# luliic2/rttnw

Measured on NVIDIA B200. Metric: path samples/sec, higher is better.
Workload: dtype f64

## Files before the change

rttnw_b200/csrc/api.cu:

```cuda
#include <cuda_runtime.h>
#include <dlfcn.h>

#include <cmath>
#include <cstdio>
#include <cstdlib>
#include <cstring>
#include <mutex>
#include <algorithm>
#include <chrono>
#include <condition_variable>
#include <deque>
#include <functional>
#include <thread>
#include <new>
#include <string>
#include <vector>

#include "../../include/rttnw_b200.h"
#include "flatten.hpp"
#include "adaptive.cuh"
#include "kernels.cuh"
#include "lbvh.cuh"
#include "sah_build.cuh"
#include "shade2.cuh"
#include "trace2.cuh"
#include "trace3.cuh"
#include "scene_api.hpp"

namespace {

thread_local std::string g_err = "";

int fail(int code, const std::string& msg) {
    g_err = msg;
    return code;
// ... 10 lines not shown

struct ArenaSlot {
    void* p;
    size_t bytes;
};
struct ArraySlot {
    cudaArray_t arr;
    cudaTextureObject_t tex;
    int w, h;
};
struct DeviceCache {
    std::mutex m;
    std::vector<ArenaSlot> arenas;
    std::vector<ArraySlot> arrays;
};
constexpr int kMaxDevices = 64;
constexpr size_t kCacheKeep = 4;
DeviceCache g_cache[kMaxDevices];

}

struct rtx_ctx {
    int device = 0;
    cudaStream_t stream = nullptr;
    bool own_stream = false;
    int sm_count = 0;
    unsigned int* d_work_counter = nullptr;
    rtx::Counters* d_counters = nullptr;
    int node_burst = 4;
    int mode = 1;
    void* d_pool = nullptr;
    int pool_slots = 0, pool_slots_wanted = 1 << 19;
    unsigned long long* d_next_item = nullptr;
    unsigned int* d_active = nullptr;
    unsigned long long* h_status = nullptr;
    cudaEvent_t batch_done[8] = {nullptr, nullptr, nullptr, nullptr, nullptr, nullptr, nullptr, nullptr};
    int wf_batch = 8;
    int wf_wide = 0;
    int wf_streams = 2;
    int trace_form = 1;
    int trace_threads = 896;
    int t_leaf = 8, t_refill = 16, t_burst = 8;
    int order_form = 0;
    int order_groups = 512;
    void* d_order = nullptr;
    size_t order_bytes = 0;
    int smem_optin = 0;
    int prof_stride = 8;
    bool perlin_smem = true;
    bool debug_batches = false;
    int shade_form = 2;
    std::vector<cudaStream_t> aux_streams;
    std::vector<cudaEvent_t> join_events;
    cudaEvent_t fork_event = nullptr;
    unsigned long long wf_iterations = 0;
    unsigned long long launches = 0;
    int bvh_builder = 0;
    int ploc_radius = 16;
    int last_build_passes = 0;
    uint8_t* h_stage = nullptr;
    size_t stage_bytes = 0;
    bool profiling = false;
    std::vector<cudaEvent_t> prof_events;
    double prof_shade_ms = 0, prof_trace_ms = 0;
    unsigned long long prof_iterations = 0;
    int w_node = 1, w_leaf = 1, w_shade = 1;
// ... 116 lines not shown
    c->shade_form = env_int("RTX_SHADE", c->shade_form);
    c->debug_batches = env_int("RTX_DEBUG_BATCHES", 0) != 0;
    if (const char* v = std::getenv("RTX_PERLIN_SMEM")) c->perlin_smem = std::atoi(v) != 0;
    c->prof_stride = env_int("RTX_PROF_STRIDE", c->prof_stride);
    if (const char* v = std::getenv("RTX_ORDER")) c->order_form = std::atoi(v);
    c->order_groups = env_int("RTX_ORDER_GROUPS", c->order_groups);
    { int g = 8; while (g * 2 <= c->order_groups && g < (1 << 15)) g *= 2; c->order_groups = g; }
    cudaDeviceGetAttribute(&c->smem_optin, cudaDevAttrMaxSharedMemoryPerBlockOptin, device);
    if (const char* m = std::getenv("RTX_MODE")) c->mode = std::strcmp(m, "mega") == 0 ? 0 : 1;
    if (const char* m = std::getenv("RTX_BVH"))
        c->bvh_builder = std::strcmp(m, "lbvh") == 0 ? 1 : (std::strcmp(m, "ploc") == 0 ? 2 : (std::strcmp(m, "sah_device") == 0 ? 3 : 0));
    c->ploc_radius = env_int("RTX_PLOC_RADIUS", c->ploc_radius);
    cudaFuncSetCacheConfig(rtx::render_kernel<false>, cudaFuncCachePreferL1);
    cudaFuncSetCacheConfig(rtx::trace_rays_kernel<false>, cudaFuncCachePreferL1);
    *out = c;
    return RTX_OK;
}

int rtx_ctx_destroy(rtx_ctx* c) {
    if (!c) return RTX_OK;
    if (c->worker.joinable()) {
        join_async(c);
        { std::lock_guard<std::mutex> lock(c->mu); c->stop = true; }
        c->cv.notify_all();
        c->worker.join();
    }
    cudaSetDevice(c->device);
    if (c->stream || !c->own_stream) cudaStreamSynchronize(c->stream);
    cudaFree(c->d_work_counter);
    cudaFree(c->d_counters);
    cudaFree(c->d_pool);
    cudaFree(c->d_order);
    cudaFree(c->d_next_item);
    cudaFree(c->d_active);
    if (c->h_status) cudaFreeHost(c->h_status);
    if (c->h_stage) cudaFreeHost(c->h_stage);
    for (auto& e : c->batch_done)
        if (e) cudaEventDestroy(e);
    for (auto e : c->prof_events) cudaEventDestroy(e);
    for (auto e : c->join_events) cudaEventDestroy(e);
    for (auto st : c->aux_streams) cudaStreamDestroy(st);
    if (c->fork_event) cudaEventDestroy(c->fork_event);
    if (c->own_stream) cudaStreamDestroy(c->stream);
    delete c;
    return RTX_OK;
}

int rtx_ctx_set_async(rtx_ctx* c, int on) {
    if (!c) return fail(RTX_ERR_INVALID, "ctx is NULL");
    JOIN(c);
    c->async = on != 0;
    if (c->async && !c->worker.joinable()) c->worker = std::thread(worker_main, c);
    return RTX_OK;
}

int rtx_ctx_sync(rtx_ctx* c) {
    if (!c) return fail(RTX_ERR_INVALID, "ctx is NULL");
    JOIN(c);
    CU(cudaSetDevice(c->device));
    CU(cudaStreamSynchronize(c->stream));
    return RTX_OK;
}
void* rtx_ctx_stream(rtx_ctx* c) { return c ? (void*)c->stream : nullptr; }
int rtx_ctx_set_profiling(rtx_ctx* c, int on) {
    if (!c) return fail(RTX_ERR_INVALID, "ctx is NULL");
    c->profiling = on != 0;
// ... 350 lines not shown

int rtx_trace_rays_stats(rtx_ctx* c, const rtx_scene* s, int64_t n, const rtx_ray* d_rays, rtx_trace_stats* out) {
    if (!c || !s || n <= 0 || !d_rays || !out) return fail(RTX_ERR_INVALID, "bad argument");
    JOIN(c);
    CU(cudaSetDevice(c->device));
    CU(cudaMemsetAsync(c->d_counters, 0, sizeof(rtx::Counters), c->stream));
    const int block = 128;
    int64_t grid = (n + block - 1) / block;
    if (grid > 0x7fffffff) return fail(RTX_ERR_INVALID, "too many rays for one launch");
    rtx::trace_rays_kernel<true><<<(unsigned)grid, block, 0, c->stream>>>(s->view, n, d_rays, nullptr, c->d_counters);
    c->launches += 1;
    CU(cudaGetLastError());
    rtx::Counters h;
    CU(cudaMemcpyAsync(&h, c->d_counters, sizeof(h), cudaMemcpyDeviceToHost, c->stream));
    CU(cudaStreamSynchronize(c->stream));
    double dn = (double)n;
    out->rays = dn;
    out->box_tests = (double)h.box_tests / dn;
    out->node_visits = (double)h.node_visits / dn;
    out->sphere_tests = (double)h.sphere_tests / dn;
    out->rect_tests = (double)h.rect_tests / dn;
    out->instance_enters = (double)h.instance_enters / dn;
    out->medium_tests = (double)h.medium_tests / dn;
    return RTX_OK;
}

static size_t order_bins_padded(int groups) {
    const size_t unit = 4 * (size_t)rtx::kShadeBlock;
    return ((size_t)8 * (size_t)groups + 1 + unit - 1) / unit * unit;
}
static int wf_prepare(rtx_ctx* c, int64_t slots) {
    if (slots > c->pool_slots) {
        if (c->d_pool) { CU(cudaStreamSynchronize(c->stream)); CU(cudaFree(c->d_pool)); c->d_pool = nullptr; c->pool_slots = 0; }
        CU(cudaMalloc(&c->d_pool, (size_t)slots * rtx::kPoolBytesPerSlot + 256));
        c->pool_slots = (int)slots;
    }
    if (c->order_form != 0) {
        const size_t bins = order_bins_padded(c->order_groups);
        const size_t need = (size_t)c->wf_streams * ((2 * bins + 64) * 4) + (size_t)slots * 12 + 4096;
        if (need > c->order_bytes) {
            if (c->d_order) { CU(cudaStreamSynchronize(c->stream)); CU(cudaFree(c->d_order)); c->d_order = nullptr; c->order_bytes = 0; }
            CU(cudaMalloc(&c->d_order, need));
            c->order_bytes = need;
        }
    }
    if (!c->d_next_item) CU(cudaMalloc(&c->d_next_item, sizeof(unsigned long long)));
    if (!c->d_active) CU(cudaMalloc(&c->d_active, 8 * sizeof(unsigned int)));

    if (!c->h_status) CU(cudaMallocHost(&c->h_status, 16 * sizeof(unsigned long long)));
    while ((int)c->aux_streams.size() < c->wf_streams - 1) {
        cudaStream_t st;
        cudaEvent_t ev;
        CU(cudaStreamCreateWithFlags(&st, cudaStreamNonBlocking));
        CU(cudaEventCreateWithFlags(&ev, cudaEventDisableTiming));
        c->aux_streams.push_back(st);
        c->join_events.push_back(ev);
    }
    if (!c->fork_event) CU(cudaEventCreateWithFlags(&c->fork_event, cudaEventDisableTiming));
    for (auto& e : c->batch_done)
        if (!e) CU(cudaEventCreateWithFlags(&e, cudaEventDisableTiming));
    return RTX_OK;
}

static int render_wavefront(rtx_ctx* c, const rtx_scene* s, const rtx_render_params* p, float* d_accum,
                            unsigned long long* d_ray_count, bool counted, const uint32_t* tile_list = nullptr,
                            int64_t n_list = 0, float* d_aux = nullptr) {
    const bool adaptive = tile_list != nullptr;
    const int64_t n_tiles = adaptive ? n_list : (int64_t)((p->width + rtx::kTileW - 1) / rtx::kTileW) * ((p->height + rtx::kTileH - 1) / rtx::kTileH);
    const unsigned long long total = (unsigned long long)n_tiles * 32ull * (unsigned long long)p->spp_count;
    int64_t slots = c->pool_slots_wanted;
    if ((unsigned long long)slots > total / 24) slots = (int64_t)(total / 24);
    if (slots < (256 << 10)) slots = 256 << 10;
    if (slots > c->pool_slots_wanted) slots = c->pool_slots_wanted;
    if ((unsigned long long)slots > total) slots = (int64_t)total;
    slots = (slots + rtx::kWfBlock - 1) / rtx::kWfBlock * rtx::kWfBlock;
    int rc = wf_prepare(c, slots);
    if (rc != RTX_OK) return rc;
    rtx::WfArgs a;
    a.sc = s->view;
    a.cam = s->camera;
    a.width = p->width; a.height = p->height;
    a.spp_begin = p->spp_begin; a.spp_count = p->spp_count; a.max_depth = p->max_depth;
    a.k0 = (uint32_t)p->seed; a.k1 = (uint32_t)(p->seed >> 32);
    a.tiles_x = (p->width + rtx::kTileW - 1) / rtx::kTileW;
    a.tiles_y = (p->height + rtx::kTileH - 1) / rtx::kTileH;
    a.inv_per_block_row = 1.0f / (float)(a.tiles_x * rtx::kBlockH);
    a.n_slots = (int32_t)slots;
    a.total_items = total;
    a.next_item = c->d_next_item;
    a.adaptive.tile_list = tile_list;
    a.adaptive.aux = reinterpret_cast<float4*>(d_aux);
    {
        uint8_t* base = (uint8_t*)c->d_pool;
        size_t n = (size_t)slots;
        double** d8[8] = {&a.pool.ox, &a.pool.oy, &a.pool.oz, &a.pool.dx, &a.pool.dy, &a.pool.dz, &a.pool.time, &a.pool.best_t};
        for (auto pp : d8) { *pp = (double*)base; base += n * 8; }
        a.pool.best_rec = (int32_t*)base; base += n * 4;
        a.pool.best_chain = (int32_t*)base; base += n * 4;
        a.pool.bounce = (int32_t*)base; base += n * 4;
        a.pool.pixel = (uint32_t*)base; base += n * 4;
        a.pool.sample = (uint32_t*)base; base += n * 4;
        float** f4[3] = {&a.pool.thr_r, &a.pool.thr_g, &a.pool.thr_b};
        for (auto pp : f4) { *pp = (float*)base; base += n * 4; }
    }
    CU(cudaMemsetAsync(a.pool.bounce, 0xFF, (size_t)slots * 4, c->stream));
    CU(cudaMemsetAsync(c->d_next_item, 0, sizeof(unsigned long long), c->stream));
    float4* acc = reinterpret_cast<float4*>(d_accum);
    const int batch = c->wf_batch;
    const bool wide = c->wf_wide != 0 && s->view.wide_root >= 0;
    const int P = (slots >= (int64_t)c->wf_streams * 4 * rtx::kWfBlock) ? c->wf_streams : 1;
    const bool ordered = c->order_form != 0 && c->shade_form >= 2 && c->trace_form == 1 && !wide;
    if (ordered) CU(cudaMemsetAsync(c->d_order, 0, (size_t)P * (2 * order_bins_padded(c->order_groups) + 64) * 4, c->stream));
    struct Part {
        rtx::WfArgs a;
        cudaStream_t stream;
        unsigned grid, sgrid;
        bool done;
    };
    std::vector<Part> parts((size_t)P);
    {
        int64_t per = slots / P / rtx::kWfBlock * rtx::kWfBlock;
        for (int q = 0; q < P; ++q) {
            Part& pt = parts[(size_t)q];
            int64_t begin = (int64_t)q * per, count = q == P - 1 ? slots - begin : per;
            pt.a = a;
            pt.a.n_slots = (int32_t)count;
            double** d8[8] = {&pt.a.pool.ox, &pt.a.pool.oy, &pt.a.pool.oz, &pt.a.pool.dx, &pt.a.pool.dy, &pt.a.pool.dz, &pt.a.pool.time, &pt.a.pool.best_t};
            for (auto pp : d8) *pp += begin;
            pt.a.pool.best_rec += begin; pt.a.pool.best_chain += begin; pt.a.pool.bounce += begin;
            pt.a.pool.pixel += begin; pt.a.pool.sample += begin;
            float** f4[3] = {&pt.a.pool.thr_r, &pt.a.pool.thr_g, &pt.a.pool.thr_b};
            for (auto pp : f4) *pp += begin;
            if (ordered) {
                const size_t bins = order_bins_padded(c->order_groups);
                uint32_t* w = (uint32_t*)c->d_order + (size_t)q * (2 * bins + 64);
                rtx::OrderArgs& o = pt.a.order;
                o.hist = w;
                o.offsets = w + bins;
                o.done = w + 2 * bins + 1;
                uint8_t* per_slot = (uint8_t*)c->d_order + (((size_t)P * (2 * bins + 64) * 4 + 255) & ~(size_t)255);
                o.key_rank = (uint2*)per_slot + begin;
                o.order = (uint32_t*)(per_slot + (size_t)slots * 8) + begin;
                o.n_bins_padded = (int32_t)bins;
                o.groups = c->order_groups;
                o.shift = 0;
                while (((s->n_records - 1) >> o.shift) >= o.groups) ++o.shift;
            }
            pt.grid = (unsigned)(count / rtx::kTraceBlock);
            pt.sgrid = (unsigned)(count / rtx::kShadeBlock);
            pt.done = false;
            pt.stream = q == 0 ? c->stream : c->aux_streams[(size_t)q - 1];
        }
        if (P > 1) {
            CU(cudaEventRecord(c->fork_event, c->stream));
            for (int q = 1; q < P; ++q) CU(cudaStreamWaitEvent(parts[(size_t)q].stream, c->fork_event, 0));
        }
    }
    rtx::TraceCfg tcfg{};
    int t2_threads = 0;
    size_t t2_smem = 0;
    unsigned t2_grid_cap = (unsigned)c->sm_count;
    if (c->trace_form >= 2 && !wide && s->world_node_count > 0 && s->world_depth <= rtx::kShortStack) {
        t2_threads = c->trace_threads >= 1024 ? 1024 : c->trace_threads >= 896 ? 896 : (c->trace_threads >= 640 ? 640 : (c->trace_threads >= 512 ? 512 : 448));
        const size_t stack_bytes = (size_t)(1 + rtx::kShortStack) * (size_t)t2_threads * 4 + 16;
        const size_t room = (size_t)c->smem_optin > stack_bytes ? (size_t)c->smem_optin - stack_bytes : 0;
        int cap = (int)std::min<size_t>(room / rtx::kNodeStride, (size_t)s->world_node_count);
        if (cap < 1) {
            t2_threads = 0;
        } else {
            tcfg.stage_first = s->world_first_node;
            tcfg.n_stage = cap;
            tcfg.cap = cap;
            tcfg.t_leaf = c->t_leaf; tcfg.t_refill = c->t_refill; tcfg.burst = c->t_burst;
            t2_smem = (size_t)cap * rtx::kNodeStride + stack_bytes;
        }
    }
    rtx::Trace3Cfg t3cfg{};
    int t3_threads = 0;
    size_t t3_smem = 0;
    if (c->trace_form == 3 && !wide && s->world_node_count > 0 && s->world_depth <= rtx::kShortStack) {
        t3_threads = c->trace_threads >= 896 ? 896 : (c->trace_threads >= 768 ? 768 : (c->trace_threads >= 640 ? 640 : 512));
        const size_t fixed = rtx::trace3_smem_bytes(t3_threads, 0);
        const size_t room = (size_t)c->smem_optin > fixed ? (size_t)c->smem_optin - fixed : 0;
        const int cap = (int)std::min<size_t>(room / rtx::kNodeStride, (size_t)s->world_node_count);
        if (cap < 1) {
            t3_threads = 0;
        } else {
            t3cfg.stage_first = s->world_first_node;
            t3cfg.n_stage = cap;
            t3cfg.cap = cap;
            t3cfg.burst = c->t_burst;
            t3_smem = rtx::trace3_smem_bytes(t3_threads, cap);
            t2_threads = 0;
        }
    }
    const bool t1c = c->trace_form == 4 && !wide && s->world_depth <= rtx::kShortStack;
    if (t1c) t2_threads = 0;
    const bool t3_all = t3_threads != 0 && t3cfg.n_stage == s->world_node_count;
    auto launch_trace3 = [&](const Part& pt) -> cudaError_t {
        unsigned grid = std::min<unsigned>((unsigned)c->sm_count, (unsigned)((pt.a.n_slots + t3_threads - 1) / t3_threads));
        if (grid < 1) grid = 1;
#define RTX_T3_LAUNCH(CNT, THR, ALL)                                                                                               \
    do {                                                                                                                           \
        auto k = rtx::wf_trace3_kernel<CNT, THR, ALL>;                                                                             \
        cudaError_t e = cudaFuncSetAttribute(k, cudaFuncAttributeMaxDynamicSharedMemorySize, (int)t3_smem);                         \
        if (e != cudaSuccess) return e;                                                                                            \
        k<<<grid, THR, t3_smem, pt.stream>>>(pt.a.sc, pt.a.pool, pt.a.n_slots, t3cfg, d_ray_count, CNT ? c->d_counters : nullptr); \
    } while (0)
#define RTX_T3_THREADS(CNT, ALL)                                  \
    do {                                                          \
        if (t3_threads == 896) RTX_T3_LAUNCH(CNT, 896, ALL);      \
        else if (t3_threads == 768) RTX_T3_LAUNCH(CNT, 768, ALL); \
        else if (t3_threads == 640) RTX_T3_LAUNCH(CNT, 640, ALL); \
        else RTX_T3_LAUNCH(CNT, 512, ALL);                        \
    } while (0)
        if (counted) { if (t3_all) RTX_T3_THREADS(true, true); else RTX_T3_THREADS(true, false); }
        else { if (t3_all) RTX_T3_THREADS(false, true); else RTX_T3_THREADS(false, false); }
#undef RTX_T3_THREADS
#undef RTX_T3_LAUNCH
        return cudaSuccess;
    };
    const bool t2_all = t2_threads != 0 && tcfg.n_stage == s->world_node_count;
    auto launch_trace2 = [&](const Part& pt) -> cudaError_t {
        unsigned grid = std::min<unsigned>(t2_grid_cap, (unsigned)((pt.a.n_slots + t2_threads - 1) / t2_threads));
        if (grid < 1) grid = 1;
#define RTX_T2_LAUNCH(CNT, THR, ALL)                                                                                              \
    do {                                                                                                                          \
        auto k = rtx::wf_trace2_kernel<CNT, THR, ALL>;                                                                            \
        cudaError_t e = cudaFuncSetAttribute(k, cudaFuncAttributeMaxDynamicSharedMemorySize, (int)t2_smem);                        \
        if (e != cudaSuccess) return e;                                                                                           \
        k<<<grid, THR, t2_smem, pt.stream>>>(pt.a.sc, pt.a.pool, pt.a.n_slots, tcfg, d_ray_count, CNT ? c->d_counters : nullptr); \
// ... 3 lines not shown
        if (t2_threads == 1024) RTX_T2_LAUNCH(CNT, 1024, ALL);    \
        else if (t2_threads == 896) RTX_T2_LAUNCH(CNT, 896, ALL); \
        else if (t2_threads == 640) RTX_T2_LAUNCH(CNT, 640, ALL); \
        else if (t2_threads == 512) RTX_T2_LAUNCH(CNT, 512, ALL); \
        else RTX_T2_LAUNCH(CNT, 448, ALL);                        \
    } while (0)
        if (counted) { if (t2_all) RTX_T2_THREADS(true, true); else RTX_T2_THREADS(true, false); }
        else { if (t2_all) RTX_T2_THREADS(false, true); else RTX_T2_THREADS(false, false); }
#undef RTX_T2_THREADS
#undef RTX_T2_LAUNCH
        return cudaSuccess;
    };
    size_t prof_used = 0;
    const int kProfStride = c->prof_stride;
    long long iteration = 0;
    bool prof_now = false;
    auto prof_mark = [&](void) -> cudaError_t {
        if (!prof_now) return cudaSuccess;
        if (prof_used == c->prof_events.size()) {
            cudaEvent_t e;
            cudaError_t err = cudaEventCreate(&e);
            if (err != cudaSuccess) return err;
            c->prof_events.push_back(e);
        }
        return cudaEventRecord(c->prof_events[prof_used++], c->stream);
    };
    int remaining = P;
    for (int k = 0; remaining > 0; ++k) {
        const int par = k & 1;
        for (int q = 0; q < P; ++q) {
            Part& pt = parts[(size_t)q];
            if (pt.done) continue;
            unsigned int* d_act = c->d_active + 2 * q + par;
            for (int it = 0; it < batch; ++it) {
                unsigned int* active = nullptr;
                if (it == batch - 1) {
                    active = d_act;
                    CU(cudaMemsetAsync(active, 0, sizeof(unsigned int), pt.stream));
                }
                prof_now = q == 0 && c->profiling && (iteration++ % kProfStride) == 0;
                CU(prof_mark());
                if (adaptive) {
                    if (c->perlin_smem && s->n_perlins == 1) rtx::wf_shade2_kernel<false, true, false, true><<<pt.sgrid, rtx::kShadeBlock, 0, pt.stream>>>(pt.a, acc, active, nullptr);
                    else rtx::wf_shade2_kernel<false, false, false, true><<<pt.sgrid, rtx::kShadeBlock, 0, pt.stream>>>(pt.a, acc, active, nullptr);
                } else if (c->shade_form >= 2) {
                    if (counted && !ordered) rtx::wf_shade2_kernel<true><<<pt.sgrid, rtx::kShadeBlock, 0, pt.stream>>>(pt.a, acc, active, c->d_counters);
                    else if (ordered) {
                        if (counted) rtx::wf_shade2_kernel<true, false, true><<<pt.sgrid, rtx::kShadeBlock, 0, pt.stream>>>(pt.a, acc, active, c->d_counters);
                        else if (c->perlin_smem && s->n_perlins == 1) rtx::wf_shade2_kernel<false, true, true><<<pt.sgrid, rtx::kShadeBlock, 0, pt.stream>>>(pt.a, acc, active, nullptr);
                        else rtx::wf_shade2_kernel<false, false, true><<<pt.sgrid, rtx::kShadeBlock, 0, pt.stream>>>(pt.a, acc, active, nullptr);
                        rtx::wf_order_kernel<<<(unsigned)((pt.a.n_slots + 255) / 256), 256, 0, pt.stream>>>(pt.a.order, pt.a.n_slots);
                    }
                    else if (c->perlin_smem && s->n_perlins == 1) rtx::wf_shade2_kernel<false, true><<<pt.sgrid, rtx::kShadeBlock, 0, pt.stream>>>(pt.a, acc, active, nullptr);
                    else rtx::wf_shade2_kernel<false><<<pt.sgrid, rtx::kShadeBlock, 0, pt.stream>>>(pt.a, acc, active, nullptr);
                } else {
                    if (counted) rtx::wf_shade_kernel<true><<<pt.sgrid, rtx::kShadeBlock, 0, pt.stream>>>(pt.a, acc, active, c->d_counters);
                    else rtx::wf_shade_kernel<false><<<pt.sgrid, rtx::kShadeBlock, 0, pt.stream>>>(pt.a, acc, active, nullptr);
                }
                CU(prof_mark());
                CU(prof_mark());
                if (ordered) {
                    if (counted) rtx::wf_trace_ordered_kernel<true><<<pt.grid, rtx::kTraceBlock, 0, pt.stream>>>(pt.a.sc, pt.a.pool, pt.a.order, d_ray_count, c->d_counters);
                    else rtx::wf_trace_ordered_kernel<false><<<pt.grid, rtx::kTraceBlock, 0, pt.stream>>>(pt.a.sc, pt.a.pool, pt.a.order, d_ray_count, nullptr);
                } else if (t1c) {
                    if (counted) rtx::wf_trace1c_kernel<true><<<pt.grid, rtx::kTraceBlock, 0, pt.stream>>>(pt.a.sc, pt.a.pool, pt.a.n_slots, d_ray_count, c->d_counters);
                    else rtx::wf_trace1c_kernel<false><<<pt.grid, rtx::kTraceBlock, 0, pt.stream>>>(pt.a.sc, pt.a.pool, pt.a.n_slots, d_ray_count, nullptr);
                } else if (t3_threads != 0) {
                    CU(launch_trace3(pt));
                } else if (t2_threads != 0) {
                    CU(launch_trace2(pt));
                } else if (counted) {
                    if (wide)
                        rtx::wf_trace_kernel<true, true><<<pt.grid, rtx::kTraceBlock, 0, pt.stream>>>(pt.a.sc, pt.a.pool, pt.a.n_slots, d_ray_count, c->d_counters);
                    else
                        rtx::wf_trace_kernel<true><<<pt.grid, rtx::kTraceBlock, 0, pt.stream>>>(pt.a.sc, pt.a.pool, pt.a.n_slots, d_ray_count, c->d_counters);
                } else {
                    if (wide)
                        rtx::wf_trace_kernel<false, true><<<pt.grid, rtx::kTraceBlock, 0, pt.stream>>>(pt.a.sc, pt.a.pool, pt.a.n_slots, d_ray_count, nullptr);
                    else
                        rtx::wf_trace_kernel<false><<<pt.grid, rtx::kTraceBlock, 0, pt.stream>>>(pt.a.sc, pt.a.pool, pt.a.n_slots, d_ray_count, nullptr);
                }
                CU(prof_mark());
            }
            CU(cudaGetLastError());
            c->launches += (ordered ? 3ull : 2ull) * (unsigned long long)batch;
            if (q == 0) c->wf_iterations += (unsigned long long)batch;
            unsigned long long* hs = c->h_status + 4 * q + 2 * par;
            hs[0] = 0;
            CU(cudaMemcpyAsync(&hs[0], d_act, sizeof(unsigned int), cudaMemcpyDeviceToHost, pt.stream));
            CU(cudaMemcpyAsync(&hs[1], c->d_next_item, sizeof(unsigned long long), cudaMemcpyDeviceToHost, pt.stream));
            CU(cudaEventRecord(c->batch_done[2 * q + par], pt.stream));
        }
        if (k >= 1) {
            const int prev = par ^ 1;
            for (int q = 0; q < P; ++q) {
                Part& pt = parts[(size_t)q];
                if (pt.done) continue;
                CU(cudaEventSynchronize(c->batch_done[2 * q + prev]));
                const unsigned long long* hs = c->h_status + 4 * q + 2 * prev;
                if (c->debug_batches) std::fprintf(stderr, "[rtx] batch %d partition %d: %u rays written by its last shade pass, dispenser at %llu of %llu\n", k - 1, q, (unsigned int)hs[0], hs[1], total);
                if ((unsigned int)hs[0] == 0 && hs[1] >= total) { pt.done = true; --remaining; }
            }
        }
    }
    if (P > 1)
        for (int q = 1; q < P; ++q) {
            CU(cudaEventRecord(c->join_events[(size_t)q - 1], parts[(size_t)q].stream));
            CU(cudaStreamWaitEvent(c->stream, c->join_events[(size_t)q - 1], 0));
        }
    if (c->profiling && prof_used >= 4) {
        CU(cudaEventSynchronize(c->prof_events[prof_used - 1]));
        for (size_t q = 0; q + 3 < prof_used; q += 4) {
            float ms = 0.f;
            CU(cudaEventElapsedTime(&ms, c->prof_events[q], c->prof_events[q + 1]));
            c->prof_shade_ms += ms * kProfStride;
            CU(cudaEventElapsedTime(&ms, c->prof_events[q + 2], c->prof_events[q + 3]));
            c->prof_trace_ms += ms * kProfStride;
            c->prof_iterations += kProfStride;
        }
    }
    return RTX_OK;
}

static int render_launch(rtx_ctx* c, const rtx_scene* s, const rtx_render_params* p, float* d_accum,
                         unsigned long long* d_ray_count, bool counted) {
    if (!c || !s || !p || !d_accum) return fail(RTX_ERR_INVALID, "NULL argument");
    if (p->width <= 0 || p->height <= 0 || p->spp_count < 0 || p->spp_begin < 0 || p->max_depth < 0)
        return fail(RTX_ERR_INVALID, "bad render parameters");
    if ((int64_t)p->width * p->height > 0x7fffffff) return fail(RTX_ERR_INVALID, "image too large");
    if (p->spp_count > (1 << 24)) return fail(RTX_ERR_INVALID, "more than 2^24 samples per pixel in one call (the fp32 sample count of the accumulator)");
    if (p->spp_count == 0) return RTX_OK;
    CU(cudaSetDevice(c->device));
    if (p->max_depth == 0) {
        int n = p->width * p->height;
// ... 525 lines not shown
```

rttnw_b200/csrc/kernels.cuh:

```cuda
#pragma once
#ifndef K1_MINB
#define K1_MINB 5
#endif
#include <cuda_runtime.h>
#include <math_constants.h>
#include <stdint.h>

#include "../../include/rttnw_b200.h"
#include "device_types.h"
#include "order.cuh"

namespace rtx {

__device__ __forceinline__ double ldg_d(const double* p) { return __ldg(p); }

struct d3 {
    double x, y, z;
};
__device__ __forceinline__ d3 mk(double x, double y, double z) { return d3{x, y, z}; }
__device__ __forceinline__ d3 operator+(d3 a, d3 b) { return mk(a.x + b.x, a.y + b.y, a.z + b.z); }
__device__ __forceinline__ d3 operator-(d3 a, d3 b) { return mk(a.x - b.x, a.y - b.y, a.z - b.z); }
__device__ __forceinline__ d3 operator*(double s, d3 a) { return mk(s * a.x, s * a.y, s * a.z); }
__device__ __forceinline__ d3 operator-(d3 a) { return mk(-a.x, -a.y, -a.z); }
__device__ __forceinline__ double dot(d3 a, d3 b) { return a.x * b.x + a.y * b.y + a.z * b.z; }
// ... 995 lines not shown
                pending = 0;
                st = ST_TRAV;
                ++my_rays;
            }
        }
    }
    if (ray_count) {
        for (int off = 16; off > 0; off >>= 1) my_rays += __shfl_xor_sync(FULL, my_rays, off);
        if (lane == 0 && my_rays) atomicAdd(ray_count, my_rays);
    }
    if constexpr (kCount) {
        uint32_t vals[4] = {tally.n_node, tally.n_sphere, tally.n_rect, tally.n_med};
#pragma unroll
        for (int k = 0; k < 4; ++k)
            for (int off = 16; off > 0; off >>= 1) vals[k] += __shfl_xor_sync(FULL, vals[k], off);
        if (lane == 0) {
            atomicAdd(&counters->node_visits, (unsigned long long)vals[0]);
            atomicAdd(&counters->box_tests, 2ull * vals[0]);
            atomicAdd(&counters->sphere_tests, (unsigned long long)vals[1]);
            atomicAdd(&counters->rect_tests, (unsigned long long)vals[2]);
            atomicAdd(&counters->medium_tests, (unsigned long long)vals[3]);
        }
    }
}

struct PathPool {
    double *ox, *oy, *oz, *dx, *dy, *dz, *time, *best_t;
    int32_t *best_rec, *best_chain, *bounce;
    uint32_t *pixel, *sample;
    float *thr_r, *thr_g, *thr_b;
};
constexpr int kPoolBytesPerSlot = 8 * 8 + 8 * 4;

struct AdaptiveArgs {
    const uint32_t* tile_list;
    float4* aux;
};

struct WfArgs {
    SceneView sc;
    CameraView cam;
    PathPool pool;
    int32_t width, height, spp_begin, spp_count, max_depth;
    uint32_t k0, k1;
    int32_t tiles_x, tiles_y;
    float inv_per_block_row;
    int32_t n_slots;
    unsigned long long total_items;
    unsigned long long* next_item;
    union {
        OrderArgs order;
        AdaptiveArgs adaptive;
    };
};

constexpr int kWfBlock = 128;
#ifndef WF_SHADE_BLOCK
#define WF_SHADE_BLOCK 128
#endif
constexpr int kShadeBlock = WF_SHADE_BLOCK;
#ifndef WF_TRACE_BLOCK
#define WF_TRACE_BLOCK 128
#endif
constexpr int kTraceBlock = WF_TRACE_BLOCK;
#ifndef WF_TRACE_MINB
#define WF_TRACE_MINB 7
#endif
#ifndef WF_SHADE_MINB
#define WF_SHADE_MINB 5
#endif

template <bool kCount>
__global__ void __launch_bounds__(kShadeBlock, WF_SHADE_MINB * (128 / kShadeBlock)) wf_shade_kernel(WfArgs a, float4* __restrict__ accum, unsigned int* active_out, Counters* counters) {
    const unsigned FULL = 0xffffffffu;
    const int tid = threadIdx.x;
    const int lane = tid & 31;
    const int i = blockIdx.x * blockDim.x + tid;
    const bool valid = i < a.n_slots;
    int32_t stack[kStackSize];
    Tally<kCount> tally;

    int bounce = valid ? a.pool.bounce[i] : -2;
// ... 55 lines not shown
                }
            }
        }
    }

    if (fresh) {
        smp.bounce = (uint32_t)bounce;
        Best best{1.7976931348623157e308, -1, 0};
        if (a.sc.n_media > 0) {
            SlabRay sr;
            make_slab(ray.o, ray.d, sr);
            media_prepass<false>(a.sc, ray, sr, 0.001, best, 0.0, &smp, stack, tally);
        }
        a.pool.ox[i] = ray.o.x; a.pool.oy[i] = ray.o.y; a.pool.oz[i] = ray.o.z;
        a.pool.dx[i] = ray.d.x; a.pool.dy[i] = ray.d.y; a.pool.dz[i] = ray.d.z;
        a.pool.time[i] = ray.time;
        a.pool.best_t[i] = best.t; a.pool.best_rec[i] = best.rec; a.pool.best_chain[i] = best.chain;
        a.pool.thr_r[i] = pc.thr_r; a.pool.thr_g[i] = pc.thr_g; a.pool.thr_b[i] = pc.thr_b;
        a.pool.pixel[i] = smp.pixel; a.pool.sample[i] = smp.sample;
        a.pool.bounce[i] = bounce;
    }
    if (active_out) {
        const unsigned am = __ballot_sync(FULL, fresh);
        if (lane == 0 && am != 0) atomicAdd(active_out, (unsigned int)__popc(am));
    }
    if constexpr (kCount) {
        uint32_t v = tally.n_med;
        for (int off = 16; off > 0; off >>= 1) v += __shfl_xor_sync(FULL, v, off);
        if (lane == 0 && v) atomicAdd(&counters->medium_tests, (unsigned long long)v);
    }
}

template <bool kCount, bool kWide = false>
__global__ void __launch_bounds__(kTraceBlock, WF_TRACE_MINB * (128 / kTraceBlock)) wf_trace_kernel(SceneView sc, PathPool pool, int n_slots, unsigned long long* ray_count,
                                                            Counters* counters) {
    const unsigned FULL = 0xffffffffu;
    const int lane = threadIdx.x & 31;
    const int i = blockIdx.x * blockDim.x + threadIdx.x;
    int32_t stack[kStackSize];
    Tally<kCount> tally;
    const bool act = i < n_slots && pool.bounce[i] >= 0;
    if (act) {
        RayD ray{mk(pool.ox[i], pool.oy[i], pool.oz[i]), mk(pool.dx[i], pool.dy[i], pool.dz[i]), pool.time[i]};
        Best best{pool.best_t[i], -1, 0};
        if constexpr (kWide) traverse_wide(sc, sc.wide_root, ray, 0.001, best, stack, tally);
        else traverse_simple(sc, sc.world_root, ray, 0.001, best, stack, 0, tally);
        if (best.rec >= 0) {
            pool.best_t[i] = best.t;
            pool.best_rec[i] = best.rec;
            pool.best_chain[i] = best.chain;
        }
    }
    if (ray_count) {
        const unsigned am = __ballot_sync(FULL, act);
        if (lane == 0 && am != 0) atomicAdd(ray_count, (unsigned long long)__popc(am));
    }
    if constexpr (kCount) {
        uint32_t vals[3] = {tally.n_node, tally.n_sphere, tally.n_rect};
#pragma unroll
        for (int k = 0; k < 3; ++k)
            for (int off = 16; off > 0; off >>= 1) vals[k] += __shfl_xor_sync(FULL, vals[k], off);
        if (lane == 0) {
            atomicAdd(&counters->node_visits, (unsigned long long)vals[0]);
            atomicAdd(&counters->box_tests, 2ull * vals[0]);
            atomicAdd(&counters->sphere_tests, (unsigned long long)vals[1]);
            atomicAdd(&counters->rect_tests, (unsigned long long)vals[2]);
        }
    }
}

template <bool kCount>
__global__ void __launch_bounds__(kTraceBlock, WF_TRACE_MINB * (128 / kTraceBlock)) wf_trace_ordered_kernel(SceneView sc, PathPool pool, OrderArgs o, unsigned long long* ray_count,
                                                                                                              Counters* counters) {
    const unsigned FULL = 0xffffffffu;
// ... 104 lines not shown
```

rttnw_b200/csrc/shade2.cuh:

```cuda
#pragma once
#include "kernels.cuh"

namespace rtx {

template <bool kCount>
__device__ __forceinline__ void media_after(const SceneView& sc, const RayD& ray, double tmin, Best& best, const Sampler& smp,
                                            int32_t* stack, Tally<kCount>& tally) {
    const float dx = (float)ray.d.x, dy = (float)ray.d.y, dz = (float)ray.d.z;
    const float len_ub = sqrtf(fmaf(dx, dx, fmaf(dy, dy, dz * dz))) * 1.000001f;
    const float seg_ub = (__double2float_ru(best.t) - __double2float_rd(tmin)) * len_ub * 1.000001f;
    uint4 w = make_uint4(0, 0, 0, 0);
    int32_t w_block = -1;
    bool have_slab = false;
    SlabRay s;
    for (int32_t m = 0; m < sc.n_media; ++m) {
        const float4* mp = reinterpret_cast<const float4*>(sc.media + m);
        const float4 lo = __ldg(mp), hi = __ldg(mp + 1);
        const float inv_density_lb = __ldg(reinterpret_cast<const float*>(mp + 2));
        const int32_t ord = __float_as_int(hi.w);
        if ((ord >> 2) != w_block) {
            w_block = ord >> 2;
            w = smp.block(P_MEDIUM, (uint32_t)w_block);
        }
        const uint32_t word = (ord & 3) == 0 ? w.x : ((ord & 3) == 1 ? w.y : ((ord & 3) == 2 ? w.z : w.w));
        const float flight_lb = inv_density_lb * (-logf(u01f(word))) * 0.999999f;
        if (flight_lb > seg_ub) continue;
        if (!have_slab) {
            make_slab(ray.o, ray.d, s);
            have_slab = true;
        }
        float tn;
        if (!slab(s, lo.x, hi.x, lo.y, hi.y, lo.z, hi.z, __double2float_rd(tmin), __double2float_ru(best.t), tn)) continue;
        const int32_t ri = __float_as_int(lo.w);
        double t;
        if (medium_candidate<false>(sc, ri, ray, tmin, best.t, u01d(word), stack, t, tally)) {
            best.t = t;
            best.rec = ri;
            best.chain = 0;
        }
    }
}

template <bool kCount, bool kPerlinShared = false, bool kOrder = false, bool kAdaptive = false>
__global__ void __launch_bounds__(kShadeBlock, WF_SHADE_MINB*(128 / kShadeBlock)) wf_shade2_kernel(WfArgs a, float4* __restrict__ accum, unsigned int* active_out,
                                                                                                   Counters* counters) {
    const unsigned FULL = 0xffffffffu;
    const int tid = threadIdx.x;
    const int lane = tid & 31;
    const int i = blockIdx.x * blockDim.x + tid;
    const bool valid = i < a.n_slots;
    int32_t stack[kStackSize];
    Tally<kCount> tally;

    int bounce = valid ? a.pool.bounce[i] : -2;
    const bool dry = __ldcg(a.next_item) >= a.total_items;
    if constexpr (kPerlinShared) {
        __shared__ DPerlin s_perlin;
        static_assert(sizeof(DPerlin) % 16 == 0, "DPerlin is copied in 16-byte words");
        const uint4* src = reinterpret_cast<const uint4*>(a.sc.perlins);
        uint4* dst = reinterpret_cast<uint4*>(&s_perlin);
        for (int k = tid; k < (int)(sizeof(DPerlin) / 16); k += kShadeBlock) dst[k] = __ldg(src + k);
        __syncthreads();
        a.sc.perlins = &s_perlin;
    }

    RayD ray{mk(0, 0, 0), mk(0, 0, 1), 0.0};
    PathColor pc{1.f, 1.f, 1.f, 0.f, 0.f, 0.f};
    Sampler smp{a.k0, a.k1, 0u, 0u, 0u};
    bool fresh = false;
    int32_t src_rec = -1;
    if (bounce >= 0) {
        ray.o = mk(a.pool.ox[i], a.pool.oy[i], a.pool.oz[i]);
        ray.d = mk(a.pool.dx[i], a.pool.dy[i], a.pool.dz[i]);
        ray.time = a.pool.time[i];
        Best best{a.pool.best_t[i], a.pool.best_rec[i], a.pool.best_chain[i]};
        pc = PathColor{a.pool.thr_r[i], a.pool.thr_g[i], a.pool.thr_b[i], 0.f, 0.f, 0.f};
        smp.pixel = a.pool.pixel[i];
        smp.sample = a.pool.sample[i];
        smp.bounce = (uint32_t)bounce;
        if (a.sc.n_media > 0) media_after(a.sc, ray, 0.001, best, smp, stack, tally);
        Albedo al;
        const bool ended = shade_hit<false, kPerlinShared>(a.sc, a.cam.background, a.max_depth, ray, best, smp, pc, bounce, al);
        apply_albedo(pc, al);
        if (ended) {
            atomicAdd(accum + smp.pixel, make_float4(pc.rad_r, pc.rad_g, pc.rad_b, 1.0f));
            if constexpr (kAdaptive)
                if (smp.sample & 1u) atomicAdd(a.adaptive.aux + smp.pixel, make_float4(pc.rad_r, pc.rad_g, pc.rad_b, 1.0f));
            bounce = -1;
            a.pool.bounce[i] = -1;
        } else {
            fresh = true;
            src_rec = best.rec;
        }
    }
    {
        const bool want = bounce == -1;
        unsigned m = dry ? 0u : __ballot_sync(FULL, want);
        if (m != 0) {
            const int leader = __ffs(m) - 1;
            unsigned long long base = 0;
            if (lane == leader) base = atomicAdd(a.next_item, (unsigned long long)__popc(m));
            base = __shfl_sync(FULL, base, leader);
            const unsigned long long item = base + (unsigned long long)__popc(m & ((1u << lane) - 1u));
            if (want && item < a.total_items) {
                const unsigned long long group = item >> 5;
                const unsigned int tile = (unsigned int)(group / (unsigned long long)a.spp_count);
                const unsigned int smp_i = (unsigned int)(group - (unsigned long long)tile * (unsigned long long)a.spp_count);
                int tx, ty;
                tile_of_order(kAdaptive ? __ldg(a.adaptive.tile_list + tile) : tile, a.tiles_x, a.tiles_y, a.inv_per_block_row, tx, ty);
                const int pi = (int)(item & 31ull);
                const int px = tx * kTileW + (pi & (kTileW - 1));
                const int row = ty * kTileH + (pi / kTileW);
                if (px < a.width && row < a.height) {
                    smp.pixel = (uint32_t)(row * a.width + px);
                    smp.sample = (uint32_t)a.spp_begin + smp_i;
                    smp.bounce = 0;
                    camera_ray(a.cam, a.width, a.height, px, a.height - 1 - row, smp, ray);
                    pc = PathColor{1.f, 1.f, 1.f, 0.f, 0.f, 0.f};
                    bounce = 0;
                    fresh = true;
                }
            }
        }
    }
    if (fresh) {
        a.pool.ox[i] = ray.o.x; a.pool.oy[i] = ray.o.y; a.pool.oz[i] = ray.o.z;
        a.pool.dx[i] = ray.d.x; a.pool.dy[i] = ray.d.y; a.pool.dz[i] = ray.d.z;
        a.pool.time[i] = ray.time;
        a.pool.best_t[i] = 1.7976931348623157e308; a.pool.best_rec[i] = -1; a.pool.best_chain[i] = 0;
        a.pool.thr_r[i] = pc.thr_r; a.pool.thr_g[i] = pc.thr_g; a.pool.thr_b[i] = pc.thr_b;
        a.pool.pixel[i] = smp.pixel; a.pool.sample[i] = smp.sample;
        a.pool.bounce[i] = bounce;
    }
    if constexpr (kOrder) {
        uint2 kr = make_uint2(kOrderDead, 0u);
        if (fresh) kr.x = order_key(a.order, src_rec, ray.d.x, ray.d.y, ray.d.z);
        {
            const unsigned same = __match_any_sync(FULL, kr.x);
            const int leader = __ffs(same) - 1;
            uint32_t base = 0;
            if (fresh && lane == leader) base = atomicAdd(a.order.hist + kr.x, (uint32_t)__popc(same));
            base = __shfl_sync(FULL, base, leader);
            kr.y = base + (uint32_t)__popc(same & ((1u << lane) - 1u));
        }
        if (valid) a.order.key_rank[i] = kr;
        order_scan_by_last_cta<kShadeBlock>(a.order, tid);
    }
    if (active_out) {
        const unsigned am = __ballot_sync(FULL, fresh);
        if (lane == 0 && am != 0) atomicAdd(active_out, (unsigned int)__popc(am));
    }
    if constexpr (kCount) {
        uint32_t v = tally.n_med;
        for (int off = 16; off > 0; off >>= 1) v += __shfl_xor_sync(FULL, v, off);
        if (lane == 0 && v) atomicAdd(&counters->medium_tests, (unsigned long long)v);
    }
}

}
```

Measured before the change: 628.6 million.

## Compact live paths into a double-buffered pool during the wavefront drain tail

Doubles the path pool into two halves. Once the work dispenser runs dry, the shade kernel stream-compacts the surviving paths into the other half with a warp-aggregated atomic counter, and a small device-side DrainState records which half and how many paths are live. Trace and shade kernels read this view and exit early for blocks past the live count. The host also shrinks the launch grids using the live count read back from the previous batch. This is meant to stop the tail iterations from launching and scanning the mostly dead full pool, at the cost of twice the pool memory, volatile loads of the drain state, and more complex cross-kernel ordering.

```diff
diff --git a/rttnw_b200/csrc/api.cu b/rttnw_b200/csrc/api.cu
--- a/rttnw_b200/csrc/api.cu
+++ b/rttnw_b200/csrc/api.cu
@@ -1,6 +1,7 @@
 #include <cuda_runtime.h>
 #include <dlfcn.h>
 
+#include <climits>
 #include <cmath>
 #include <cstdio>
 #include <cstdlib>
@@ -77,6 +78,7 @@
     void* d_pool = nullptr;
     int pool_slots = 0, pool_slots_wanted = 1 << 19;
     unsigned long long* d_next_item = nullptr;
+    rtx::DrainState* d_drain = nullptr;
     unsigned int* d_active = nullptr;
     unsigned long long* h_status = nullptr;
     cudaEvent_t batch_done[8] = {nullptr, nullptr, nullptr, nullptr, nullptr, nullptr, nullptr, nullptr};
@@ -259,6 +261,7 @@
     cudaFree(c->d_pool);
     cudaFree(c->d_order);
     cudaFree(c->d_next_item);
+    cudaFree(c->d_drain);
     cudaFree(c->d_active);
     if (c->h_status) cudaFreeHost(c->h_status);
     if (c->h_stage) cudaFreeHost(c->h_stage);
@@ -675,7 +678,7 @@
 static int wf_prepare(rtx_ctx* c, int64_t slots) {
     if (slots > c->pool_slots) {
         if (c->d_pool) { CU(cudaStreamSynchronize(c->stream)); CU(cudaFree(c->d_pool)); c->d_pool = nullptr; c->pool_slots = 0; }
-        CU(cudaMalloc(&c->d_pool, (size_t)slots * rtx::kPoolBytesPerSlot + 256));
+        CU(cudaMalloc(&c->d_pool, 2 * (size_t)slots * rtx::kPoolBytesPerSlot + 256));
         c->pool_slots = (int)slots;
     }
     if (c->order_form != 0) {
@@ -688,6 +691,7 @@
         }
     }
     if (!c->d_next_item) CU(cudaMalloc(&c->d_next_item, sizeof(unsigned long long)));
+    if (!c->d_drain) CU(cudaMalloc(&c->d_drain, 4 * sizeof(rtx::DrainState)));
     if (!c->d_active) CU(cudaMalloc(&c->d_active, 8 * sizeof(unsigned int)));
 
     if (!c->h_status) CU(cudaMallocHost(&c->h_status, 16 * sizeof(unsigned long long)));
@@ -735,7 +739,7 @@
     a.adaptive.aux = reinterpret_cast<float4*>(d_aux);
     {
         uint8_t* base = (uint8_t*)c->d_pool;
-        size_t n = (size_t)slots;
+        size_t n = 2 * (size_t)slots;
         double** d8[8] = {&a.pool.ox, &a.pool.oy, &a.pool.oz, &a.pool.dx, &a.pool.dy, &a.pool.dz, &a.pool.time, &a.pool.best_t};
         for (auto pp : d8) { *pp = (double*)base; base += n * 8; }
         a.pool.best_rec = (int32_t*)base; base += n * 4;
@@ -746,7 +750,7 @@
         float** f4[3] = {&a.pool.thr_r, &a.pool.thr_g, &a.pool.thr_b};
         for (auto pp : f4) { *pp = (float*)base; base += n * 4; }
     }
-    CU(cudaMemsetAsync(a.pool.bounce, 0xFF, (size_t)slots * 4, c->stream));
+    CU(cudaMemsetAsync(a.pool.bounce, 0xFF, 2 * (size_t)slots * 4, c->stream));
     CU(cudaMemsetAsync(c->d_next_item, 0, sizeof(unsigned long long), c->stream));
     float4* acc = reinterpret_cast<float4*>(d_accum);
     const int batch = c->wf_batch;
@@ -754,11 +758,16 @@
     const int P = (slots >= (int64_t)c->wf_streams * 4 * rtx::kWfBlock) ? c->wf_streams : 1;
     const bool ordered = c->order_form != 0 && c->shade_form >= 2 && c->trace_form == 1 && !wide;
     if (ordered) CU(cudaMemsetAsync(c->d_order, 0, (size_t)P * (2 * order_bins_padded(c->order_groups) + 64) * 4, c->stream));
+    CU(cudaMemsetAsync(c->d_drain, 0, (size_t)P * sizeof(rtx::DrainState), c->stream));
     struct Part {
         rtx::WfArgs a;
         cudaStream_t stream;
         unsigned grid, sgrid;
         bool done;
+        long long pass;
+        long long batch_end[2];
+        long long small_from;
+        unsigned bound;
     };
     std::vector<Part> parts((size_t)P);
     {
@@ -768,12 +777,14 @@
             int64_t begin = (int64_t)q * per, count = q == P - 1 ? slots - begin : per;
             pt.a = a;
             pt.a.n_slots = (int32_t)count;
+            pt.a.drain = c->d_drain + q;
+            const int64_t at = 2 * begin;
             double** d8[8] = {&pt.a.pool.ox, &pt.a.pool.oy, &pt.a.pool.oz, &pt.a.pool.dx, &pt.a.pool.dy, &pt.a.pool.dz, &pt.a.pool.time, &pt.a.pool.best_t};
-            for (auto pp : d8) *pp += begin;
-            pt.a.pool.best_rec += begin; pt.a.pool.best_chain += begin; pt.a.pool.bounce += begin;
-            pt.a.pool.pixel += begin; pt.a.pool.sample += begin;
+            for (auto pp : d8) *pp += at;
+            pt.a.pool.best_rec += at; pt.a.pool.best_chain += at; pt.a.pool.bounce += at;
+            pt.a.pool.pixel += at; pt.a.pool.sample += at;
             float** f4[3] = {&pt.a.pool.thr_r, &pt.a.pool.thr_g, &pt.a.pool.thr_b};
-            for (auto pp : f4) *pp += begin;
+            for (auto pp : f4) *pp += at;
             if (ordered) {
                 const size_t bins = order_bins_padded(c->order_groups);
                 uint32_t* w = (uint32_t*)c->d_order + (size_t)q * (2 * bins + 64);
@@ -792,6 +803,10 @@
             pt.grid = (unsigned)(count / rtx::kTraceBlock);
             pt.sgrid = (unsigned)(count / rtx::kShadeBlock);
             pt.done = false;
+            pt.pass = 0;
+            pt.batch_end[0] = pt.batch_end[1] = -1;
+            pt.small_from = LLONG_MAX;
+            pt.bound = 0;
             pt.stream = q == 0 ? c->stream : c->aux_streams[(size_t)q - 1];
         }
         if (P > 1) {
@@ -840,6 +855,7 @@
     const bool t1c = c->trace_form == 4 && !wide && s->world_depth <= rtx::kShortStack;
     if (t1c) t2_threads = 0;
     const bool t3_all = t3_threads != 0 && t3cfg.n_stage == s->world_node_count;
+    const bool pack = c->shade_form >= 2 && !ordered && !t1c && t3_threads == 0 && t2_threads == 0;
     auto launch_trace3 = [&](const Part& pt) -> cudaError_t {
         unsigned grid = std::min<unsigned>((unsigned)c->sm_count, (unsigned)((pt.a.n_slots + t3_threads - 1) / t3_threads));
         if (grid < 1) grid = 1;
@@ -909,27 +925,44 @@
             Part& pt = parts[(size_t)q];
             if (pt.done) continue;
             unsigned int* d_act = c->d_active + 2 * q + par;
-            for (int it = 0; it < batch; ++it) {
+            for (int it = 0; it < batch; ++it, ++pt.pass) {
                 unsigned int* active = nullptr;
                 if (it == batch - 1) {
                     active = d_act;
                     CU(cudaMemsetAsync(active, 0, sizeof(unsigned int), pt.stream));
                 }
+                pt.a.par = (int32_t)(pt.pass & 1);
+                const unsigned small_s = std::max(1u, (pt.bound + rtx::kShadeBlock - 1) / rtx::kShadeBlock);
+                const unsigned small_t = std::max(1u, (pt.bound + rtx::kTraceBlock - 1) / rtx::kTraceBlock);
+                const unsigned sgrid = pt.pass >= pt.small_from ? std::min(pt.sgrid, small_s) : pt.sgrid;
+                const unsigned grid = pt.pass + 1 >= pt.small_from ? std::min(pt.grid, small_t) : pt.grid;
                 prof_now = q == 0 && c->profiling && (iteration++ % kProfStride) == 0;
                 CU(prof_mark());
                 if (adaptive) {
-                    if (c->perlin_smem && s->n_perlins == 1) rtx::wf_shade2_kernel<false, true, false, true><<<pt.sgrid, rtx::kShadeBlock, 0, pt.stream>>>(pt.a, acc, active, nullptr);
-                    else rtx::wf_shade2_kernel<false, false, false, true><<<pt.sgrid, rtx::kShadeBlock, 0, pt.stream>>>(pt.a, acc, active, nullptr);
+                    if (c->perlin_smem && s->n_perlins == 1) {
+                        auto k = pack ? rtx::wf_shade2_kernel<false, true, false, true, true> : rtx::wf_shade2_kernel<false, true, false, true>;
+                        k<<<sgrid, rtx::kShadeBlock, 0, pt.stream>>>(pt.a, acc, active, nullptr);
+                    } else {
+                        auto k = pack ? rtx::wf_shade2_kernel<false, false, false, true, true> : rtx::wf_shade2_kernel<false, false, false, true>;
+                        k<<<sgrid, rtx::kShadeBlock, 0, pt.stream>>>(pt.a, acc, active, nullptr);
+                    }
                 } else if (c->shade_form >= 2) {
-                    if (counted && !ordered) rtx::wf_shade2_kernel<true><<<pt.sgrid, rtx::kShadeBlock, 0, pt.stream>>>(pt.a, acc, active, c->d_counters);
-                    else if (ordered) {
+                    if (counted && !ordered) {
+                        auto k = pack ? rtx::wf_shade2_kernel<true, false, false, false, true> : rtx::wf_shade2_kernel<true>;
+                        k<<<sgrid, rtx::kShadeBlock, 0, pt.stream>>>(pt.a, acc, active, c->d_counters);
+                    } else if (ordered) {
                         if (counted) rtx::wf_shade2_kernel<true, false, true><<<pt.sgrid, rtx::kShadeBlock, 0, pt.stream>>>(pt.a, acc, active, c->d_counters);
                         else if (c->perlin_smem && s->n_perlins == 1) rtx::wf_shade2_kernel<false, true, true><<<pt.sgrid, rtx::kShadeBlock, 0, pt.stream>>>(pt.a, acc, active, nullptr);
                         else rtx::wf_shade2_kernel<false, false, true><<<pt.sgrid, rtx::kShadeBlock, 0, pt.stream>>>(pt.a, acc, active, nullptr);
                         rtx::wf_order_kernel<<<(unsigned)((pt.a.n_slots + 255) / 256), 256, 0, pt.stream>>>(pt.a.order, pt.a.n_slots);
                     }
-                    else if (c->perlin_smem && s->n_perlins == 1) rtx::wf_shade2_kernel<false, true><<<pt.sgrid, rtx::kShadeBlock, 0, pt.stream>>>(pt.a, acc, active, nullptr);
-                    else rtx::wf_shade2_kernel<false><<<pt.sgrid, rtx::kShadeBlock, 0, pt.stream>>>(pt.a, acc, active, nullptr);
+                    else if (c->perlin_smem && s->n_perlins == 1) {
+                        auto k = pack ? rtx::wf_shade2_kernel<false, true, false, false, true> : rtx::wf_shade2_kernel<false, true>;
+                        k<<<sgrid, rtx::kShadeBlock, 0, pt.stream>>>(pt.a, acc, active, nullptr);
+                    } else {
+                        auto k = pack ? rtx::wf_shade2_kernel<false, false, false, false, true> : rtx::wf_shade2_kernel<false>;
+                        k<<<sgrid, rtx::kShadeBlock, 0, pt.stream>>>(pt.a, acc, active, nullptr);
+                    }
                 } else {
                     if (counted) rtx::wf_shade_kernel<true><<<pt.sgrid, rtx::kShadeBlock, 0, pt.stream>>>(pt.a, acc, active, c->d_counters);
                     else rtx::wf_shade_kernel<false><<<pt.sgrid, rtx::kShadeBlock, 0, pt.stream>>>(pt.a, acc, active, nullptr);
@@ -946,19 +979,15 @@
                     CU(launch_trace3(pt));
                 } else if (t2_threads != 0) {
                     CU(launch_trace2(pt));
-                } else if (counted) {
-                    if (wide)
-                        rtx::wf_trace_kernel<true, true><<<pt.grid, rtx::kTraceBlock, 0, pt.stream>>>(pt.a.sc, pt.a.pool, pt.a.n_slots, d_ray_count, c->d_counters);
-                    else
-                        rtx::wf_trace_kernel<true><<<pt.grid, rtx::kTraceBlock, 0, pt.stream>>>(pt.a.sc, pt.a.pool, pt.a.n_slots, d_ray_count, c->d_counters);
                 } else {
-                    if (wide)
-                        rtx::wf_trace_kernel<false, true><<<pt.grid, rtx::kTraceBlock, 0, pt.stream>>>(pt.a.sc, pt.a.pool, pt.a.n_slots, d_ray_count, nullptr);
-                    else
-                        rtx::wf_trace_kernel<false><<<pt.grid, rtx::kTraceBlock, 0, pt.stream>>>(pt.a.sc, pt.a.pool, pt.a.n_slots, d_ray_count, nullptr);
+                    auto k = counted ? (wide ? rtx::wf_trace_kernel<true, true> : rtx::wf_trace_kernel<true>)
+                                     : (wide ? rtx::wf_trace_kernel<false, true> : rtx::wf_trace_kernel<false>);
+                    k<<<grid, rtx::kTraceBlock, 0, pt.stream>>>(pt.a.sc, pt.a.pool, pt.a.n_slots, pt.a.drain, pt.a.par, d_ray_count,
+                                                                counted ? c->d_counters : nullptr);
                 }
                 CU(prof_mark());
             }
+            pt.batch_end[par] = pt.pass - 1;
             CU(cudaGetLastError());
             c->launches += (ordered ? 3ull : 2ull) * (unsigned long long)batch;
             if (q == 0) c->wf_iterations += (unsigned long long)batch;
@@ -977,6 +1006,10 @@
                 const unsigned long long* hs = c->h_status + 4 * q + 2 * prev;
                 if (c->debug_batches) std::fprintf(stderr, "[rtx] batch %d partition %d: %u rays written by its last shade pass, dispenser at %llu of %llu\n", k - 1, q, (unsigned int)hs[0], hs[1], total);
                 if ((unsigned int)hs[0] == 0 && hs[1] >= total) { pt.done = true; --remaining; }
+                if (pack && hs[1] >= total) {
+                    pt.bound = (unsigned int)hs[0];
+                    if (pt.small_from == LLONG_MAX) pt.small_from = pt.batch_end[prev] + 3;
+                }
             }
         }
     }
diff --git a/rttnw_b200/csrc/kernels.cuh b/rttnw_b200/csrc/kernels.cuh
--- a/rttnw_b200/csrc/kernels.cuh
+++ b/rttnw_b200/csrc/kernels.cuh
@@ -1051,6 +1051,45 @@
 };
 constexpr int kPoolBytesPerSlot = 8 * 8 + 8 * 4;
 
+struct DrainView {
+    uint32_t pack;
+    uint32_t src;
+    uint32_t packed;
+    uint32_t live;
+};
+struct DrainState {
+    DrainView view[2];
+    uint32_t count[2];
+    uint32_t dry;
+    uint32_t pad;
+};
+
+__device__ __forceinline__ int32_t ld_early(const int32_t* p) {
+    int32_t v;
+    asm volatile("ld.volatile.global.s32 %0, [%1];" : "=r"(v) : "l"(p));
+    return v;
+}
+__device__ __forceinline__ unsigned long long ld_early_cg(const unsigned long long* p) {
+    unsigned long long v;
+    asm volatile("ld.volatile.global.u64 %0, [%1];" : "=l"(v) : "l"(p));
+    return v;
+}
+__device__ __forceinline__ uint4 ld_view(const DrainState* d, int p) {
+    uint4 v;
+    asm volatile("ld.volatile.global.v4.u32 {%0, %1, %2, %3}, [%4];" : "=r"(v.x), "=r"(v.y), "=r"(v.z), "=r"(v.w) : "l"(&d->view[p]));
+    return v;
+}
+
+__device__ __forceinline__ void drain_trace_view(DrainState* d, int p, int32_t n_slots, uint32_t& half, int32_t& live) {
+    const uint4 v = ld_view(d, p);
+    half = v.x ? v.y ^ 1u : v.y;
+    live = v.x ? (int32_t)__ldcg(&d->count[p]) : (v.z ? (int32_t)v.w : n_slots);
+    if (blockIdx.x == 0 && threadIdx.x == 0) {
+        *reinterpret_cast<uint4*>(&d->view[p ^ 1]) = make_uint4(__ldcg(&d->dry), half, v.x, (uint32_t)live);
+        d->count[p ^ 1] = 0;
+    }
+}
+
 struct AdaptiveArgs {
     const uint32_t* tile_list;
     float4* aux;
@@ -1067,6 +1106,8 @@
     int32_t n_slots;
     unsigned long long total_items;
     unsigned long long* next_item;
+    DrainState* drain;
+    int32_t par;
     union {
         OrderArgs order;
         AdaptiveArgs adaptive;
@@ -1188,14 +1229,22 @@
 }
 
 template <bool kCount, bool kWide = false>
-__global__ void __launch_bounds__(kTraceBlock, WF_TRACE_MINB * (128 / kTraceBlock)) wf_trace_kernel(SceneView sc, PathPool pool, int n_slots, unsigned long long* ray_count,
-                                                            Counters* counters) {
+__global__ void __launch_bounds__(kTraceBlock, WF_TRACE_MINB * (128 / kTraceBlock)) wf_trace_kernel(SceneView sc, PathPool pool, int n_slots, DrainState* drain, int par,
+                                                                                                    unsigned long long* ray_count, Counters* counters) {
     const unsigned FULL = 0xffffffffu;
     const int lane = threadIdx.x & 31;
-    const int i = blockIdx.x * blockDim.x + threadIdx.x;
+    const int s = blockIdx.x * blockDim.x + threadIdx.x;
+    const int sl = s < n_slots ? s : 0;
+    const int32_t b0 = ld_early(pool.bounce + sl), b1 = ld_early(pool.bounce + n_slots + sl);
+    uint32_t half;
+    int32_t live;
+    drain_trace_view(drain, par, n_slots, half, live);
+    if (blockIdx.x * blockDim.x >= live) return;
+    const int i = half ? s + n_slots : s;
+    const int bounce = half ? b1 : b0;
     int32_t stack[kStackSize];
     Tally<kCount> tally;
-    const bool act = i < n_slots && pool.bounce[i] >= 0;
+    const bool act = s < live && bounce >= 0;
     if (act) {
         RayD ray{mk(pool.ox[i], pool.oy[i], pool.oz[i]), mk(pool.dx[i], pool.dy[i], pool.dz[i]), pool.time[i]};
         Best best{pool.best_t[i], -1, 0};
diff --git a/rttnw_b200/csrc/shade2.cuh b/rttnw_b200/csrc/shade2.cuh
--- a/rttnw_b200/csrc/shade2.cuh
+++ b/rttnw_b200/csrc/shade2.cuh
@@ -41,19 +41,36 @@
     }
 }
 
-template <bool kCount, bool kPerlinShared = false, bool kOrder = false, bool kAdaptive = false>
+template <bool kCount, bool kPerlinShared = false, bool kOrder = false, bool kAdaptive = false, bool kPack = false>
 __global__ void __launch_bounds__(kShadeBlock, WF_SHADE_MINB*(128 / kShadeBlock)) wf_shade2_kernel(WfArgs a, float4* __restrict__ accum, unsigned int* active_out,
                                                                                                    Counters* counters) {
+    static_assert(!(kOrder && kPack), "the ordered trace pass reads the pool in place");
     const unsigned FULL = 0xffffffffu;
     const int tid = threadIdx.x;
     const int lane = tid & 31;
-    const int i = blockIdx.x * blockDim.x + tid;
-    const bool valid = i < a.n_slots;
+    const int s = blockIdx.x * blockDim.x + tid;
+    const bool valid = s < a.n_slots;
     int32_t stack[kStackSize];
     Tally<kCount> tally;
 
-    int bounce = valid ? a.pool.bounce[i] : -2;
-    const bool dry = __ldcg(a.next_item) >= a.total_items;
+    int bounce;
+    bool dry;
+    int i = s;
+    int pack_to = -1;
+    if constexpr (kPack) {
+        const int sl = valid ? s : 0;
+        const int32_t b0 = ld_early(a.pool.bounce + sl), b1 = ld_early(a.pool.bounce + a.n_slots + sl);
+        dry = ld_early_cg(a.next_item) >= a.total_items;
+        const uint4 v = ld_view(a.drain, a.par);
+        const int32_t live = v.z ? (int32_t)v.w : a.n_slots;
+        if (blockIdx.x * blockDim.x >= live) return;
+        if (v.y) i = s + a.n_slots;
+        bounce = s >= live ? -2 : (v.y ? b1 : b0);
+        if (v.x) pack_to = v.y ? 0 : a.n_slots;
+    } else {
+        bounce = valid ? a.pool.bounce[s] : -2;
+        dry = __ldcg(a.next_item) >= a.total_items;
+    }
     if constexpr (kPerlinShared) {
         __shared__ DPerlin s_perlin;
         static_assert(sizeof(DPerlin) % 16 == 0, "DPerlin is copied in 16-byte words");
@@ -95,6 +112,8 @@
     }
     {
         const bool want = bounce == -1;
+        if constexpr (kPack)
+            if (dry && pack_to < 0 && tid == 0) a.drain->dry = 1u;
         unsigned m = dry ? 0u : __ballot_sync(FULL, want);
         if (m != 0) {
             const int leader = __ffs(m) - 1;
@@ -123,14 +142,25 @@
             }
         }
     }
+    int w = i;
+    if constexpr (kPack) {
+        if (pack_to >= 0) {
+            const unsigned fm = __ballot_sync(FULL, fresh);
+            const int leader = fm ? __ffs(fm) - 1 : 0;
+            uint32_t base = 0;
+            if (lane == leader && fm) base = atomicAdd(&a.drain->count[a.par], (uint32_t)__popc(fm));
+            base = __shfl_sync(FULL, base, leader);
+            w = pack_to + (int)base + __popc(fm & ((1u << lane) - 1u));
+        }
+    }
     if (fresh) {
-        a.pool.ox[i] = ray.o.x; a.pool.oy[i] = ray.o.y; a.pool.oz[i] = ray.o.z;
-        a.pool.dx[i] = ray.d.x; a.pool.dy[i] = ray.d.y; a.pool.dz[i] = ray.d.z;
-        a.pool.time[i] = ray.time;
-        a.pool.best_t[i] = 1.7976931348623157e308; a.pool.best_rec[i] = -1; a.pool.best_chain[i] = 0;
-        a.pool.thr_r[i] = pc.thr_r; a.pool.thr_g[i] = pc.thr_g; a.pool.thr_b[i] = pc.thr_b;
-        a.pool.pixel[i] = smp.pixel; a.pool.sample[i] = smp.sample;
-        a.pool.bounce[i] = bounce;
+        a.pool.ox[w] = ray.o.x; a.pool.oy[w] = ray.o.y; a.pool.oz[w] = ray.o.z;
+        a.pool.dx[w] = ray.d.x; a.pool.dy[w] = ray.d.y; a.pool.dz[w] = ray.d.z;
+        a.pool.time[w] = ray.time;
+        a.pool.best_t[w] = 1.7976931348623157e308; a.pool.best_rec[w] = -1; a.pool.best_chain[w] = 0;
+        a.pool.thr_r[w] = pc.thr_r; a.pool.thr_g[w] = pc.thr_g; a.pool.thr_b[w] = pc.thr_b;
+        a.pool.pixel[w] = smp.pixel; a.pool.sample[w] = smp.sample;
+        a.pool.bounce[w] = bounce;
     }
     if constexpr (kOrder) {
         uint2 kr = make_uint2(kOrderDead, 0u);
```

After: 627.2 million, median of 6. About the same (-0.2%).
